# Spandan7724/Audio-Watermarking-Deep-Learning-Watermarks-for-Authenticating-Speech

Measured on AMD Instinct MI355X. Metric: 1-s@16kHz clips/sec (gen+det+loss fwd-bwd), higher is better.
Workload: dtype f32; 1 GPU; main16 train step: Generator+Detector+6 losses fwd-bwd + Adam, B=256 clips/GPU x 1 GPU, 1-s @ 16 kHz, message_bits=16 (BASELINE configs[2]); batch_per_gpu=256, global_batch=256, clip_len=16000, optimizer=fused flat Adam (wm_adam_step), parallelism=single

## Files before the change

### audio-watermarking-deep-learning-watermarks-for-authenticating-speech_amd/csrc/small_convs.hip

```cpp
#include "wm_common.hpp"
using namespace wm;

namespace {

__global__ __launch_bounds__(256) void stem_fwd_kernel(const float* __restrict__ s, const float* __restrict__ w,
                                                       const float* __restrict__ bias, float* __restrict__ y, int T) {
    __shared__ float ss[1024 + 8];
    __shared__ float ws[64 * 8];
    const int tilesPerClip = (T + 1023) / 1024;
    const int b = blockIdx.x / tilesPerClip, t0 = (blockIdx.x % tilesPerClip) * 1024;
    const float* sb = s + (size_t)b * T;
    for (int i = threadIdx.x; i < 1024 + 6; i += 256) {
        const int t = t0 - 3 + i;
        ss[i] = (t >= 0 && t < T) ? sb[t] : 0.f;
    }
    for (int i = threadIdx.x; i < 512; i += 256) {
        const int co = i >> 3, j = i & 7;
        ws[i] = (j < 7) ? w[co * 7 + j] : bias[co];
    }
    __syncthreads();
    const int t = t0 + 4 * threadIdx.x;
    if (t >= T) return;
    float v[10];
#pragma unroll
    for (int i = 0; i < 10; ++i) v[i] = ss[4 * threadIdx.x + i];
    float* yb = y + (size_t)b * 64 * T + t;
#pragma unroll 4
    for (int co = 0; co < 64; ++co) {
        const float* wc = ws + co * 8;
        float4 o = make_float4(wc[7], wc[7], wc[7], wc[7]);
#pragma unroll
        for (int j = 0; j < 7; ++j) {
            const float wj = wc[j];
            o.x = fmaf(wj, v[j], o.x);
            o.y = fmaf(wj, v[j + 1], o.y);
            o.z = fmaf(wj, v[j + 2], o.z);
            o.w = fmaf(wj, v[j + 3], o.w);
        }
        *reinterpret_cast<float4*>(yb + (size_t)co * T) = o;
    }
}

__global__ __launch_bounds__(256) void stem_bwd_kernel(const float* __restrict__ g, const float* __restrict__ s,
                                                       const float* __restrict__ w, float* __restrict__ ds,
                                                       float* __restrict__ partial, int B, int T, int nds) {
    constexpr int NT = 256, GS = NT + 8;
    extern __shared__ __align__(16) float smem[];
    float* gs = smem;
    float* ss = gs + 64 * GS;
    float* dsp = ss + NT + 40;
    const int tid = threadIdx.x, lane = tid & 63, wave = tid >> 6, half = lane >> 5, l31 = lane & 31;
    const int tilesPerClip = (T + NT - 1) / NT, ntiles = B * tilesPerClip;
    f32x16 acc[2];
#pragma unroll
    for (int r = 0; r < 16; ++r) { acc[0][r] = 0.f; acc[1][r] = 0.f; }
    float4 sg[16];
    float hg[2], sv[2];
    auto load_piece = [&](int tile, int p) {
        const int b = tile / tilesPerClip, t0 = (tile % tilesPerClip) * NT;
        const float* gb = g + (size_t)b * 64 * T;
        if (p < 16) {
            const int i = tid + p * 256, c = i >> 6, q = i & 63;
            sg[p] = *reinterpret_cast<const float4*>(gb + (size_t)c * T + min(t0 + 4 * q, T - 4));
            return;
        }
#pragma unroll
        for (int k = 0; k < 2; ++k) {
            const int i = min(tid + k * 256, 64 * 6 - 1), c = i / 6, h = i % 6;
            const int t = (h < 3) ? t0 - 3 + h : t0 + NT + (h - 3);
            hg[k] = gb[(size_t)c * T + min(max(t, 0), T - 1)];
            const int ts_ = t0 - 3 + tid + k * 256;
            sv[k] = s[(size_t)b * T + min(max(ts_, 0), T - 1)];
        }
    };
    auto load_tile = [&](int tile) {
#pragma unroll
        for (int p = 0; p <= 16; ++p) load_piece(tile, p);
    };
    auto write_tile = [&](int tile) {
        const int t0 = (tile % tilesPerClip) * NT;
#pragma unroll
        for (int k = 0; k < 16; ++k) {
            const int i = tid + k * 256, c = i >> 6, q = i & 63;
            float4 v = sg[k];
            if (t0 + 4 * q >= T) v = make_float4(0.f, 0.f, 0.f, 0.f);
            *reinterpret_cast<float4*>(gs + c * GS + 4 + 4 * q) = v;
        }
#pragma unroll
        for (int k = 0; k < 2; ++k) {
            const int i = tid + k * 256;
            if (i < 64 * 6) {
                const int c = i / 6, h = i % 6;
                const int t = (h < 3) ? t0 - 3 + h : t0 + NT + (h - 3);
                gs[c * GS + ((h < 3) ? 1 + h : 4 + NT + (h - 3))] = (t >= 0 && t < T) ? hg[k] : 0.f;
            }
            if (i < NT + 40) {
                const int ts_ = t0 - 3 + i;
                ss[i] = (i < NT + 6 && ts_ >= 0 && ts_ < T) ? sv[k] : 0.f;
            }
        }
    };
    int tile = blockIdx.x;
    if (tile < ntiles) load_tile(tile);
    __syncthreads();
    if (tile < ntiles) write_tile(tile);
    __syncthreads();
    while (tile < ntiles) {
        const int next = tile + gridDim.x, nextc = min(next, ntiles - 1);
        const int b = tile / tilesPerClip, t0 = (tile % tilesPerClip) * NT;
        {
            const float* ap = gs + l31 * GS + 4 + wave * 64 + half;
            const float* bp = ss + wave * 64 + half + l31;
            const bool tapcol = l31 < 7, onecol = l31 == 7;
#pragma unroll
            for (int k2 = 0; k2 < 32; ++k2) {
                if ((k2 & 1) == 0 || k2 == 31) load_piece(nextc, k2 == 31 ? 16 : k2 >> 1);
                const float sval = bp[2 * k2];
                const float bv = tapcol ? sval : (onecol ? 1.f : 0.f);
                acc[0] = mfma32(ap[2 * k2], bv, acc[0]);
                acc[1] = mfma32(ap[32 * GS + 2 * k2], bv, acc[1]);
            }
        }
        if (ds && b < nds) {
            const int cg = __builtin_amdgcn_readfirstlane(wave), tq = lane;
            float o0 = 0.f, o1 = 0.f, o2 = 0.f, o3 = 0.f;
#pragma unroll 4
            for (int cc = 0; cc < 16; ++cc) {
                const int co = cg * 16 + cc;
                const f32x4 ga = lds_read4(gs + co * GS + 4 * tq);
                const f32x4 gb4 = lds_read4(gs + co * GS + 4 * tq + 4);
                const f32x4 gc = lds_read4(gs + co * GS + 4 * tq + 8);
                const float* wc = w + co * 7;
                const float gv[10] = {ga.y, ga.z, ga.w, gb4.x, gb4.y, gb4.z, gb4.w, gc.x, gc.y, gc.z};
                const float wj[7] = {wc[0], wc[1], wc[2], wc[3], wc[4], wc[5], wc[6]};
#pragma unroll
                for (int j = 0; j < 7; ++j) {
                    o0 = fmaf(gv[6 - j], wj[j], o0); o1 = fmaf(gv[7 - j], wj[j], o1);
                    o2 = fmaf(gv[8 - j], wj[j], o2); o3 = fmaf(gv[9 - j], wj[j], o3);
                }
            }
            *reinterpret_cast<float4*>(dsp + cg * NT + 4 * tq) = make_float4(o0, o1, o2, o3);
        }
        __syncthreads();
        if (ds && b < nds) {
            const int t = t0 + tid;
            if (t < T) ds[(size_t)b * T + t] = (dsp[tid] + dsp[NT + tid]) + (dsp[2 * NT + tid] + dsp[3 * NT + tid]);
        }
        if (next < ntiles) write_tile(next);
        __syncthreads();
        tile = next;
    }
    float* red = gs;
    for (int wv = 0; wv < 4; ++wv) {
        if (wave == wv && l31 < 8) {
#pragma unroll
            for (int mt = 0; mt < 2; ++mt)
#pragma unroll
                for (int r = 0; r < 16; ++r) {
                    const int o = (mt * 32 + mfma_row(r, half)) * 8 + l31;
                    red[o] = (wv == 0) ? acc[mt][r] : red[o] + acc[mt][r];
                }
        }
        __syncthreads();
    }
    float* out = partial + (size_t)blockIdx.x * 512;
    for (int i = tid; i < 512; i += 256) out[i] = red[i];
}

__global__ __launch_bounds__(256) void reduce_partials_kernel(const float* __restrict__ partial, int nparts, int stride, int count,
                                                              float* __restrict__ out, int accumulate) {
    __shared__ double sq[4][64];
    const int i = blockIdx.x * 64 + (threadIdx.x & 63);
    const float s = (float)column_sum_d<4>(partial, nparts, (size_t)stride, i, i < count, sq);
    if (threadIdx.x < 64 && i < count) out[i] = accumulate ? out[i] + s : s;
}
__global__ __launch_bounds__(1024) void stem_reduce_kernel(const float* __restrict__ partial, int nparts, float* dw, float* db,
                                                           int accumulate) {
    __shared__ double sq[16][64];
    const int i = blockIdx.x * 64 + (threadIdx.x & 63);
    const float s = (float)column_sum_d<16>(partial, nparts, (size_t)512, i, true, sq);
    if (threadIdx.x >= 64) return;
    const int co = i >> 3, j = i & 7;
    float* dst = (j < 7) ? dw + co * 7 + j : db + co;
    *dst = accumulate ? *dst + s : s;
}

__global__ __launch_bounds__(256) void head1_fwd_kernel(const float* __restrict__ x, const float* __restrict__ w,
                                                        const float* __restrict__ bias, float* __restrict__ y, int T4,
                                                        int total4) {
    const int i = blockIdx.x * 256 + threadIdx.x;
    if (i >= total4) return;
    const int b = i / T4, q = i % T4;
    const float4* xb = reinterpret_cast<const float4*>(x) + (size_t)b * 64 * T4 + q;
    const float b0 = bias[0];
    float4 o = make_float4(b0, b0, b0, b0);
#pragma unroll 8
    for (int c = 0; c < 64; ++c) {
        const float4 v = xb[(size_t)c * T4];
        const float wc = w[c];
        o.x = fmaf(wc, v.x, o.x); o.y = fmaf(wc, v.y, o.y); o.z = fmaf(wc, v.z, o.z); o.w = fmaf(wc, v.w, o.w);
    }
    reinterpret_cast<float4*>(y)[i] = o;
}

template <bool MASK>
__global__ __launch_bounds__(256) void head1_tail_fwd_kernel(const float* __restrict__ x, const float* __restrict__ y2,
                                                             const float* __restrict__ scale, const float* __restrict__ shift,
                                                             float* __restrict__ out, unsigned* __restrict__ mask,
                                                             const float* __restrict__ w, const float* __restrict__ bias,
                                                             float* __restrict__ y, int T4) {
    const int tilesPerClip = (T4 + 255) / 256;
    const int b = blockIdx.x / tilesPerClip, q = (blockIdx.x % tilesPerClip) * 256 + (int)threadIdx.x;
    const bool ok = q < T4;
// ... 110 lines not shown
            unsigned* mrow = mask + ((size_t)b * 64 + lane) * nw;
            if (w0 < nw) mrow[w0] = mlo;
            if (w0 + 1 < nw) mrow[w0 + 1] = mhi;
        }
    } else {
#pragma unroll
        for (int c = 0; c < 64; ++c) v[c] = x[base + (size_t)c * T];
    }
    float sl = 0.f, sb = 0.f, yl = 0.f;
    long long msg = 0;
    if constexpr (LOSS) {
        if (b < BL) { msg = message[b]; yl = 1.f; }
    }
    auto one_output = [&](int o) {
        const float* wo = w + o * 64;
        float a0 = bias[o], a1 = 0.f, a2 = 0.f, a3 = 0.f;
#pragma unroll
        for (int c = 0; c < 64; c += 4) {
            a0 = fmaf(wo[c], v[c], a0); a1 = fmaf(wo[c + 1], v[c + 1], a1);
            a2 = fmaf(wo[c + 2], v[c + 2], a2); a3 = fmaf(wo[c + 3], v[c + 3], a3);
        }
        const float lg = (a0 + a1) + (a2 + a3);
        os[threadIdx.x * OS + o] = lg;
        if constexpr (LOSS) {
            const float term = valid ? bce_logits(lg, o == 0 ? yl : (float)((msg >> ((o - 1) & 63)) & 1)) : 0.f;
            if (o == 0) sl += term;
            else if (b < BL) sb += term;
        }
    };
    if constexpr (NOC > 0) {
#pragma unroll
        for (int o = 0; o < NOC; ++o) one_output(o);
    } else {
#pragma unroll 1
        for (int o = 0; o < no; ++o) {
            __builtin_amdgcn_sched_barrier(0);
            one_output(o);
        }
    }
    __syncthreads();
    const int nvalid = min(256, T - t0) * NO;
    float* yb = y + ((size_t)b * T + t0) * NO;
    for (int i = threadIdx.x; i < nvalid; i += 256) {
        if constexpr (NOC > 0) yb[i] = os[i];
        else { const int r = div_small(i, magic); yb[i] = os[r * OS + (i - r * NO)]; }
    }
    if constexpr (LOSS) {
        sl = block_sum<4>(sl, scratch);
        sb = block_sum<4>(sb, scratch + 4);
        if (threadIdx.x == 0) { partial[blockIdx.x] = sl; partial[gridDim.x + blockIdx.x] = sb; }
    }
}

template <int NOC, int NT, bool DL>
__global__ __launch_bounds__(256) void headN_bwd_kernel(const float* __restrict__ g, const float* __restrict__ x,
                                                        const float* __restrict__ w, float* __restrict__ dx,
                                                        float* __restrict__ partial, int B, int T, int no, unsigned magic,
                                                        const long long* __restrict__ message, const float* __restrict__ g_loc,
                                                        const float* __restrict__ g_bce, int BL) {
    constexpr int XS = 257, OB = 32 * NT, GS = OB + 1;
    constexpr int NOMAX = NOC > 0 ? NOC : OB;
    const int NO = NOC > 0 ? NOC : no;
    const int KS = (NO + 1) / 2;
    float kl = 0.f, kb = 0.f;
    if constexpr (DL) {
        kl = g_loc[0] / (float)((double)B * T);
        kb = (NO > 1) ? g_bce[0] / (float)((double)BL * T * (NO - 1)) : 0.f;
    }
    extern __shared__ __align__(16) float smem[];
    float* xs = smem;
    float* gsm = xs + 64 * XS;
    float* ws = gsm + 256 * GS;
    const int tid = threadIdx.x, lane = tid & 63, wave = tid >> 6, half = lane >> 5, l31 = lane & 31;
    for (int i = tid; i < OB * 64; i += 256) ws[i] = (i < NO * 64) ? w[i] : 0.f;
    for (int i = tid; i < 256 * GS; i += 256) gsm[i] = 0.f;
    const int tilesPerClip = (T + 255) / 256, ntiles = B * tilesPerClip;
    f32x16 accw[NT][2];
#pragma unroll
    for (int mt = 0; mt < NT; ++mt)
#pragma unroll
        for (int r = 0; r < 16; ++r) { accw[mt][0][r] = 0.f; accw[mt][1][r] = 0.f; }
    float accb = 0.f;
    constexpr int NG4 = (256 * NOMAX + 3) / 4, NGV = (NG4 + 255) / 256;
    float4 sx[16], sgv[NGV];
    auto load_piece = [&](int tile, int p) {
        const int b = tile / tilesPerClip, t0 = (tile % tilesPerClip) * 256;
        if (p < 16) {
            const int i = tid + p * 256, c = i >> 6, q = i & 63;
            sx[p] = *reinterpret_cast<const float4*>(x + ((size_t)b * 64 + c) * T + min(t0 + 4 * q, T - 4));
        } else {
            const float4* gb4 = reinterpret_cast<const float4*>(g + ((size_t)b * T + t0) * NO);
            const int lim4 = ((T - t0 < 256 ? T - t0 : 256) * NO) / 4;
            sgv[p - 16] = gb4[min(tid + (p - 16) * 256, lim4 - 1)];
        }
    };
    auto load_tile = [&](int tile) {
#pragma unroll
        for (int p = 0; p < 16 + NGV; ++p) load_piece(tile, p);
    };
    auto write_tile = [&](int tile) {
        const int t0 = (tile % tilesPerClip) * 256;
        const int nt = min(256, T - t0);
        const int row = tile / tilesPerClip;
        long long msg = 0;
        if constexpr (DL) msg = (row < BL) ? message[row] : 0;
        const float yl = row < BL ? 1.f : 0.f;
#pragma unroll
        for (int k = 0; k < 16; ++k) {
            const int i = tid + k * 256, c = i >> 6, q = i & 63;
            float4 v = sx[k];
            if (4 * q >= nt) v = make_float4(0.f, 0.f, 0.f, 0.f);
            float* d = xs + c * XS + 4 * q;
            d[0] = v.x; d[1] = v.y; d[2] = v.z; d[3] = v.w;
        }
#pragma unroll
        for (int k = 0; k < NGV; ++k) {
            const int f = tid + k * 256;
            if (f < NG4) {
                const float e[4] = {sgv[k].x, sgv[k].y, sgv[k].z, sgv[k].w};
#pragma unroll
                for (int j = 0; j < 4; ++j) {
                    const int i = 4 * f + j;
                    if (i < 256 * NO) {
                        const int r = NOC > 0 ? i / NO : div_small(i, magic), o = i - r * NO;
                        float val = e[j];
                        if constexpr (DL) {
                            if (o == 0) val = bce_logits_grad(val, yl, kl);
                            else val = (row < BL) ? bce_logits_grad(val, (float)((msg >> (o - 1)) & 1), kb) : 0.f;
                        }
                        gsm[r * GS + o] = (i < nt * NO) ? val : 0.f;
                    }
                }
            }
        }
    };
    int tile = blockIdx.x;
    if (tile < ntiles) load_tile(tile);
    __syncthreads();
    if (tile < ntiles) write_tile(tile);
    __syncthreads();
    while (tile < ntiles) {
        const int next = tile + gridDim.x, nextc = min(next, ntiles - 1);
        const int b = tile / tilesPerClip, t0 = (tile % tilesPerClip) * 256;
        const int nt = min(256, T - t0);
        {
            f32x16 acc[2][2];
#pragma unroll
            for (int mt = 0; mt < 2; ++mt)
#pragma unroll
                for (int n2 = 0; n2 < 2; ++n2)
#pragma unroll
                    for (int r = 0; r < 16; ++r) acc[mt][n2][r] = 0.f;
#pragma unroll
            for (int s = 0; s < (NOMAX + 1) / 2; ++s) {
                if (s < KS) {
                    const float a0 = ws[(2 * s + half) * 64 + l31], a1 = ws[(2 * s + half) * 64 + 32 + l31];
                    const float b0 = gsm[(wave * 64 + l31) * GS + 2 * s + half], b1 = gsm[(wave * 64 + 32 + l31) * GS + 2 * s + half];
                    acc[0][0] = mfma32(a0, b0, acc[0][0]); acc[0][1] = mfma32(a0, b1, acc[0][1]);
                    acc[1][0] = mfma32(a1, b0, acc[1][0]); acc[1][1] = mfma32(a1, b1, acc[1][1]);
                }
            }
            float* dxb = dx + (size_t)b * 64 * T + t0;
#pragma unroll
            for (int mt = 0; mt < 2; ++mt)
#pragma unroll
                for (int n2 = 0; n2 < 2; ++n2)
#pragma unroll
                    for (int r = 0; r < 16; ++r) {
                        const int c = mt * 32 + mfma_row(r, half), tt = wave * 64 + n2 * 32 + l31;
                        if (tt < nt) dxb[(size_t)c * T + tt] = acc[mt][n2][r];
                    }
        }
        {
            const float* ap = gsm + (wave * 64 + half) * GS + l31;
            const float* bp = xs + l31 * XS + wave * 64 + half;
#pragma unroll
            for (int s = 0; s < 32; ++s) {
                if (s < 16 + NGV) load_piece(nextc, s);
#pragma unroll
                for (int mt = 0; mt < NT; ++mt) {
                    const float a = ap[2 * s * GS + mt * 32];
                    accw[mt][0] = mfma32(a, bp[2 * s], accw[mt][0]);
                    accw[mt][1] = mfma32(a, bp[32 * XS + 2 * s], accw[mt][1]);
                }
            }
        }
        if ((tid & (OB - 1)) < NO) {
            const float* gp = gsm + (tid / OB) * OB * GS + (tid & (OB - 1));
#pragma unroll 8
            for (int tt = 0; tt < OB; ++tt) accb += gp[tt * GS];
        }
        __syncthreads();
        if (next < ntiles) write_tile(next);
        __syncthreads();
        tile = next;
    }
    __syncthreads();
    float* red = xs;
    for (int wv = 0; wv < 4; ++wv) {
        if (wave == wv) {
#pragma unroll
            for (int mt = 0; mt < NT; ++mt)
#pragma unroll
                for (int n2 = 0; n2 < 2; ++n2)
#pragma unroll
                    for (int r = 0; r < 16; ++r) {
                        const int o = mt * 32 + mfma_row(r, half), c = n2 * 32 + l31;
                        red[o * 64 + c] = (wv == 0) ? accw[mt][n2][r] : red[o * 64 + c] + accw[mt][n2][r];
                    }
        }
        __syncthreads();
    }
    float* out = partial + (size_t)blockIdx.x * (NO * 64 + NO);
    for (int i = tid; i < NO * 64; i += 256) out[i] = red[i];
    __syncthreads();
    red[tid] = ((tid & (OB - 1)) < NO) ? accb : 0.f;
    __syncthreads();
    if (tid < NO) {
        if constexpr (NT == 1)
            out[NO * 64 + tid] = ((red[tid] + red[32 + tid]) + (red[64 + tid] + red[96 + tid])) +
                                 ((red[128 + tid] + red[160 + tid]) + (red[192 + tid] + red[224 + tid]));
        else
            out[NO * 64 + tid] = (red[tid] + red[64 + tid]) + (red[128 + tid] + red[192 + tid]);
    }
}

}

extern "C" {

int wm_stem_fwd(const float* s, const float* w, const float* bias, float* y, int B, int T, hipStream_t stream) {
    if (T & 3) return (int)hipErrorInvalidValue;
    hipLaunchKernelGGL(stem_fwd_kernel, dim3(B * ((T + 1023) / 1024)), dim3(256), 0, stream, s, w, bias, y, T);
    WM_CHECK_LAUNCH();
    return 0;
}

#ifndef WM_STEM_WGS_PER_CU
#define WM_STEM_WGS_PER_CU 2
#endif
int wm_stem_bwd(const float* g, const float* s, const float* w, float* ds, float* partial, float* dw, float* db, int B,
                int T, int nds, int accumulate, hipStream_t stream) {
    if (T & 3) return (int)hipErrorInvalidValue;
    constexpr size_t lds = (size_t)(64 * 264 + 296 + 4 * 256) * sizeof(float);
    static wm::DevOnce attr_done;
    if (int rc = wm::lds_opt_in(reinterpret_cast<const void*>(stem_bwd_kernel), lds, attr_done)) return rc;
    const int ntiles = B * ((T + 255) / 256);
    const int grid = ntiles < WM_STEM_WGS_PER_CU * kNumCU ? ntiles : WM_STEM_WGS_PER_CU * kNumCU;
    hipLaunchKernelGGL(stem_bwd_kernel, dim3(grid), dim3(256), lds, stream, g, s, w, ds, partial, B, T, nds);
    WM_CHECK_LAUNCH();
    hipLaunchKernelGGL(stem_reduce_kernel, dim3(8), dim3(1024), 0, stream, (const float*)partial, grid, dw, db, accumulate);
    WM_CHECK_LAUNCH();
    return 0;
}

int wm_head1_fwd(const float* x, const float* w, const float* bias, float* y, int B, int T, hipStream_t stream) {
    if (T & 3) return (int)hipErrorInvalidValue;
    const int total4 = B * (T / 4);
    hipLaunchKernelGGL(head1_fwd_kernel, dim3((total4 + 255) / 256), dim3(256), 0, stream, x, w, bias, y, T / 4, total4);
    WM_CHECK_LAUNCH();
    return 0;
}

int wm_head1_tail_fwd(const float* x, const float* y2, const float* scale, const float* shift, const float* w, const float* bias,
                      float* out, void* mask, float* y, int B, int T, hipStream_t stream) {
    if ((T & 3) || B <= 0 || !y2 || !out) return (int)hipErrorInvalidValue;
    const int T4 = T / 4, grid = B * ((T4 + 255) / 256);
    if (mask) hipLaunchKernelGGL(head1_tail_fwd_kernel<true>, dim3(grid), dim3(256), 0, stream, x, y2, scale, shift, out, (unsigned*)mask, w, bias, y, T4);
    else hipLaunchKernelGGL(head1_tail_fwd_kernel<false>, dim3(grid), dim3(256), 0, stream, x, y2, scale, shift, out, (unsigned*)nullptr, w, bias, y, T4);
    WM_CHECK_LAUNCH();
    return 0;
}

int wm_head1_bwd(const float* g, const float* x, const float* w, float* dx, float* partial, float* dw, float* db, int B,
                 int T, int accumulate, hipStream_t stream) {
    if (T & 3) return (int)hipErrorInvalidValue;
    const int total4 = B * (T / 4);
    int grid = (total4 + 255) / 256;
    if (grid > 1024) grid = 1024;
    if (dx) hipLaunchKernelGGL(head1_bwd_kernel<true>, dim3(grid), dim3(256), 0, stream, g, x, w, dx, partial, T / 4, total4);
    else hipLaunchKernelGGL(head1_bwd_kernel<false>, dim3(grid), dim3(256), 0, stream, g, x, w, dx, partial, T / 4, total4);
    WM_CHECK_LAUNCH();
    hipLaunchKernelGGL(reduce_partials_kernel, dim3(1), dim3(256), 0, stream, (const float*)partial, grid, 65, 64, dw, accumulate);
    WM_CHECK_LAUNCH();
    hipLaunchKernelGGL(reduce_partials_kernel, dim3(1), dim3(256), 0, stream, (const float*)partial + 64, grid, 65, 1, db, accumulate);
    WM_CHECK_LAUNCH();
    return 0;
}

}

namespace {
struct HeadNFwd {
    const float *x, *y2, *scale, *shift, *w, *bias;
    float *out, *y, *partial;
    unsigned* mask;
    const long long* message;
    int BL, R, T, NO;
};
template <int NOC, bool TAIL, bool LOSS>
int launch_headN_fwd(const HeadNFwd& a, hipStream_t stream) {
    const size_t lds = (size_t)256 * (NOC > 0 ? NOC : (a.NO | 1)) * sizeof(float);
    if constexpr (NOC == 0) {
        static wm::DevOnce done;
        if (int rc = wm::lds_opt_in(reinterpret_cast<const void*>(headN_fwd_kernel<NOC, TAIL, LOSS>), 256 * 65 * sizeof(float), done)) return rc;
    }
    const unsigned magic = (unsigned)((0x100000000ull + a.NO - 1) / a.NO);
    hipLaunchKernelGGL((headN_fwd_kernel<NOC, TAIL, LOSS>), dim3(a.R * ((a.T + 255) / 256)), dim3(256), lds, stream, a.x, a.y2, a.scale,
                       a.shift, a.out, a.mask, a.w, a.bias, a.y, a.message, a.BL, a.partial, a.T, a.NO, magic);
    WM_CHECK_LAUNCH();
    return 0;
}
template <bool TAIL, bool LOSS>
int launch_headN_fwd_width(const HeadNFwd& a, hipStream_t stream) {
    if (a.NO == 17) return launch_headN_fwd<17, TAIL, LOSS>(a, stream);
    if (a.NO == 1) return launch_headN_fwd<1, TAIL, LOSS>(a, stream);
    return launch_headN_fwd<0, TAIL, LOSS>(a, stream);
}
}

extern "C" {

int wm_headN_fwd(const float* x, const float* w, const float* bias, float* y, int B, int T, int NO, hipStream_t stream) {
    if (NO < 1 || NO > 64 || B <= 0 || T <= 0) return (int)hipErrorInvalidValue;
    const HeadNFwd a{x, nullptr, nullptr, nullptr, w, bias, nullptr, y, nullptr, nullptr, nullptr, 0, B, T, NO};
    return launch_headN_fwd_width<false, false>(a, stream);
}

int wm_headN_tail_fwd(const float* x, const float* y2, const float* scale, const float* shift, const float* w, const float* bias,
                      const long long* message, int B, float* partial, float* loc_out, float* bce_out, float* out, void* mask,
                      float* logits, int R, int T, int NO, hipStream_t stream) {
    if (NO < 1 || NO > 64 || R <= 0 || T <= 0) return (int)hipErrorInvalidValue;
    if (y2 && (!scale || !shift || !out)) return (int)hipErrorInvalidValue;
    if (message && (B < 0 || B > R || !partial || !loc_out || (NO > 1 && !bce_out))) return (int)hipErrorInvalidValue;
    const HeadNFwd a{x, y2, scale, shift, w, bias, out, logits, partial, y2 ? (unsigned*)mask : nullptr, message, B, R, T, NO};
    const int rc = y2 ? (message ? launch_headN_fwd_width<true, true>(a, stream) : launch_headN_fwd_width<true, false>(a, stream))
                      : (message ? launch_headN_fwd_width<false, true>(a, stream) : launch_headN_fwd_width<false, false>(a, stream));
    if (rc || !message) return rc;
    const int grid = R * ((T + 255) / 256);
    WM_TRY((hipError_t)wm::launch_sum_scale2(partial, grid, 1.0 / ((double)R * T), loc_out, stream));
    if (NO > 1) WM_TRY((hipError_t)wm::launch_sum_scale2(partial + grid, grid, 1.0 / ((double)B * T * (NO - 1)), bce_out, stream));
    return 0;
}

}

namespace {
struct HeadNBwd {
    const float *g, *x, *w;
    float *dx, *partial;
    const long long* message;
    const float *g_loc, *g_bce;
    int BL, R, T, NO;
};
template <int NOC, int NT, bool DL>
int launch_headN_bwd(const HeadNBwd& a, int grid, hipStream_t stream) {
    constexpr size_t lds = (size_t)(64 * 257 + 256 * (32 * NT + 1) + 32 * NT * 64) * sizeof(float);
    static wm::DevOnce done;
    if (int rc = wm::lds_opt_in(reinterpret_cast<const void*>(headN_bwd_kernel<NOC, NT, DL>), lds, done)) return rc;
    const unsigned magic = a.NO > 1 ? (unsigned)((0x100000000ull + a.NO - 1) / a.NO) : 0u;
    hipLaunchKernelGGL((headN_bwd_kernel<NOC, NT, DL>), dim3(grid), dim3(256), lds, stream, a.g, a.x, a.w, a.dx, a.partial, a.R, a.T, a.NO,
                       magic, a.message, a.g_loc, a.g_bce, a.BL);
    WM_CHECK_LAUNCH();
    return 0;
}
template <bool DL>
int headN_bwd(const HeadNBwd& a, float* dw, float* db, int accumulate, hipStream_t stream) {
    const int NO = a.NO;
    if (NO < 1 || NO > 64) return (int)hipErrorInvalidValue;
    const int ntiles = a.R * ((a.T + 255) / 256);
    const int grid = ntiles < kNumCU ? ntiles : kNumCU;
    int rc;
    if (NO == 17) rc = launch_headN_bwd<17, 1, DL>(a, grid, stream);
    else if (NO == 1) rc = launch_headN_bwd<1, 1, DL>(a, grid, stream);
    else if (NO <= 32) rc = launch_headN_bwd<0, 1, DL>(a, grid, stream);
    else rc = launch_headN_bwd<0, 2, DL>(a, grid, stream);
    if (rc) return rc;
    const int n = NO * 64 + NO;
    hipLaunchKernelGGL(reduce_partials_kernel, dim3((NO * 64 + 63) / 64), dim3(256), 0, stream, (const float*)a.partial, grid, n, NO * 64, dw, accumulate);
    WM_CHECK_LAUNCH();
    hipLaunchKernelGGL(reduce_partials_kernel, dim3(1), dim3(256), 0, stream, (const float*)a.partial + NO * 64, grid, n, NO, db, accumulate);
    WM_CHECK_LAUNCH();
    return 0;
}
}

extern "C" {

int wm_headN_bwd(const float* g, const float* x, const float* w, float* dx, float* partial, float* dw, float* db, int B,
                 int T, int NO, int accumulate, hipStream_t stream) {
    const HeadNBwd a{g, x, w, dx, partial, nullptr, nullptr, nullptr, 0, B, T, NO};
    return headN_bwd<false>(a, dw, db, accumulate, stream);
}

int wm_headN_bwd_bce(const float* logits, const long long* message, const float* g_loc, const float* g_bce, const float* x,
                     const float* w, float* dx, float* partial, float* dw, float* db, int B, int R, int T, int NO, int accumulate,
                     hipStream_t stream) {
    if (!message || !g_loc || !g_bce || B < 0 || B > R) return (int)hipErrorInvalidValue;
    const HeadNBwd a{logits, x, w, dx, partial, message, g_loc, g_bce, B, R, T, NO};
    return headN_bwd<true>(a, dw, db, accumulate, stream);
}

}
```

### audio-watermarking-deep-learning-watermarks-for-authenticating-speech_amd/csrc/wm_common.hpp

```cpp
#pragma once
#include <hip/hip_runtime.h>
#include <stdint.h>
#include <atomic>

#define WM_CHECK_LAUNCH() do { hipError_t e_ = hipGetLastError(); if (e_ != hipSuccess) return (int)e_; } while (0)
#define WM_TRY(expr) do { hipError_t e_ = (expr); if (e_ != hipSuccess) return (int)e_; } while (0)

extern "C" int wm_gscale_absmax(const float* x, long long n, float* scratch, float log2_target, float* gscale, hipStream_t stream);

namespace wm {

struct DevOnce {
    std::atomic<unsigned long long> mask{0};
};
inline bool dev_done(const DevOnce& d) {
    int dev = 0;
    if (hipGetDevice(&dev) != hipSuccess) return false;
    return (d.mask.load(std::memory_order_acquire) >> (dev & 63)) & 1ull;
}
inline void dev_mark(DevOnce& d) {
    int dev = 0;
    if (hipGetDevice(&dev) != hipSuccess) return;
    d.mask.fetch_or(1ull << (dev & 63), std::memory_order_release);
}
inline int lds_opt_in(const void* kern, size_t lds, DevOnce& once) {
    if (dev_done(once)) return 0;
    WM_TRY(hipFuncSetAttribute(kern, hipFuncAttributeMaxDynamicSharedMemorySize, (int)lds));
    dev_mark(once);
    return 0;
}

inline bool overlap(const void* a, unsigned long long na, const void* b, unsigned long long nb) {
    const uintptr_t pa = (uintptr_t)a, pb = (uintptr_t)b;
    return pa < pb + nb && pb < pa + na;
}

typedef float f32x16 __attribute__((ext_vector_type(16)));
typedef float f32x4 __attribute__((ext_vector_type(4)));

typedef const volatile __attribute__((address_space(3))) f32x4 lds_f32x4_t;
__device__ __forceinline__ f32x4 lds_read4(const float* p) { return *(lds_f32x4_t*)p; }

constexpr int kWave = 64;
constexpr int kNumCU = 256;

__device__ __forceinline__ f32x16 mfma32(float a, float b, f32x16 c) {
    return __builtin_amdgcn_mfma_f32_32x32x2f32(a, b, c, 0, 0, 0);
}
__device__ __forceinline__ int mfma_row(int r, int half) { return (r & 3) + 8 * (r >> 2) + 4 * half; }

__device__ __forceinline__ float wave_sum(float v) {
#pragma unroll
    for (int o = 32; o > 0; o >>= 1) v += __shfl_xor(v, o);
    return v;
}
__device__ __forceinline__ float half_wave_sum(float v) {
#pragma unroll
    for (int o = 16; o > 0; o >>= 1) v += __shfl_xor(v, o);
    return v;
}
__device__ __forceinline__ float half_wave_transpose_sum32(float (&x)[32], int lane) {
#pragma unroll
    for (int s = 4; s >= 0; --s) {
        const int h = 1 << s;
        const bool up = (lane >> s) & 1;
#pragma unroll
        for (int i = 0; i < h; ++i) {
            const float keep = up ? x[i + h] : x[i];
            const float send = up ? x[i] : x[i + h];
            x[i] = keep + __shfl_xor(send, h);
        }
    }
    return x[0];
}
__device__ __forceinline__ float half_wave_transpose_sum16(float (&x)[16], int lane) {
#pragma unroll
    for (int s = 3; s >= 0; --s) {
        const int h = 1 << s;
        const bool up = (lane >> s) & 1;
#pragma unroll
        for (int i = 0; i < h; ++i) {
            const float keep = up ? x[i + h] : x[i];
            const float send = up ? x[i] : x[i + h];
            x[i] = keep + __shfl_xor(send, h);
        }
    }
    return x[0] + __shfl_xor(x[0], 16);
}
__device__ __forceinline__ double wave_sum_d(double v) {
#pragma unroll
    for (int o = 32; o > 0; o >>= 1) v += __shfl_xor(v, o);
    return v;
}

template <int NW>
__device__ __forceinline__ float block_sum(float v, float* scratch) {
    v = wave_sum(v);
    const int lane = threadIdx.x & 63, w = threadIdx.x >> 6;
    __syncthreads();
    if (lane == 0) scratch[w] = v;
// ... 165 lines not shown
```

### include/wm_hip.h

```cpp
#ifndef WM_HIP_H
#define WM_HIP_H

#ifdef __cplusplus
extern "C" {
#endif

typedef struct ihipStream_t* wm_stream_t;


int wm_pack_w64(const float* w, float* wp, int KW, int mode, wm_stream_t stream);

int wm_conv64(const float* x, const float* x2, const float* wp, const float* pa, const float* pb, const float* pc,
              const float* bias, const float* e1, const float* ea, const float* eb, float* y, float* stats,
              int B, int T, int KW, int pro, int epi, wm_stream_t stream);

int wm_pack_w64_bf(const float* w, void* wpb, int mode, wm_stream_t stream);
int wm_set_conv_bf_schedule(int schedule, wm_stream_t stream);
int wm_conv64_bf(const float* x, const float* x2, const void* wpb, const float* pa, const float* pb, const float* pc,
                 const float* bias, const float* e1, const float* ea, const float* eb, float* y, float* stats,
                 int B, int T, int pro, int epi, int arith, wm_stream_t stream);
int wm_conv64_bf_tail(const float* x, const float* y2, const void* wpb_h, const float* sc2, const float* sh2, const float* bias,
                      float* out, void* mask, float* y, float* stats, int B, int T, wm_stream_t stream);

int wm_conv64_bf_stem(const float* s, const float* stem_w, const float* stem_b, const void* wpb_h, const float* bias, float* y0,
// ... 24 lines not shown
                  int arith, const float* gscale, wm_stream_t stream);
int wm_pack_w64_h7(const float* w, void* wph, int mode, wm_stream_t stream);
int wm_gscale_absmax(const float* x, long long n, float* scratch, float log2_target, float* gscale, wm_stream_t stream);
int wm_gscale_from_max(const float* maxes, int n, float log2_target, float* gscale, wm_stream_t stream);
int wm_absmax_rows(const float* x, int rows, long long row_len, float* out, wm_stream_t stream);

int wm_wgrad64_bf7(const float* g, const float* x, const float* vec, float* partial, float* dw, float* dbias, int B, int T,
                   int xpro, int accumulate, int arith, const float* gscale, wm_stream_t stream);

int wm_wgrad64_bf(const float* g, const float* g2, const float* ga, const float* gb, const float* gc,
                  const float* x, const float* xa, const float* xb, float* partial, float* dw, float* dbias,
                  int B, int T, int gpro, int xpro, int accumulate, wm_stream_t stream);

int wm_wgrad64(const float* g, const float* g2, const float* ga, const float* gb, const float* gc,
               const float* x, const float* xa, const float* xb, float* partial, float* dw, float* dbias,
               int B, int T, int KW, int gpro, int xpro, int layout, int accumulate, wm_stream_t stream);

int wm_bn_finalize(const float* partials, int nparts, double count, const float* gamma, const float* beta,
                   float* running_mean, float* running_var, long long* num_batches_tracked, float momentum, float eps,
                   float* scale, float* shift, float* save_mean, float* save_invstd, wm_stream_t stream);
int wm_bn_eval_scale_shift(const float* gamma, const float* beta, const float* running_mean, const float* running_var,
                           float eps, float* scale, float* shift, wm_stream_t stream);
int wm_bn_add_relu(const float* x, const float* y2, const float* scale, const float* shift, float* out, int B, int T,
                   wm_stream_t stream);
int wm_relu_bwd_reduce(const float* g, const float* out, const float* y2, float* dz, float* partial, int B, int T,
                       wm_stream_t stream);
int wm_bn_add_relu_mask(const float* x, const float* y2, const float* scale, const float* shift, float* out, void* mask, int B, int T,
                        wm_stream_t stream);
int wm_relu_bwd_reduce_mask(const float* g, const void* mask, const float* y2, float* dz, float* partial, float* dzmax, int B, int T,
                            wm_stream_t stream);
int wm_relu_bwd_reduce_mask_r1(const float* g1, const float* w, const void* mask, const float* y2, float* partial, float* dzmax, int B,
                               int T, wm_stream_t stream);
int wm_bn_bwd_finalize(const float* partials, int nparts, double count, const float* gamma, const float* save_mean,
                       const float* save_invstd, float* A, float* Bc, float* Cc, float* dgamma, float* dbeta,
                       int accumulate, int eval_mode, const float* dzmax, int nmax, float* gscale, wm_stream_t stream);

int wm_stem_fwd(const float* s, const float* w, const float* bias, float* y, int B, int T, wm_stream_t stream);
int wm_stem_bwd(const float* g, const float* s, const float* w, float* ds, float* partial, float* dw, float* db, int B,
                int T, int nds, int accumulate, wm_stream_t stream);
int wm_head1_fwd(const float* x, const float* w, const float* bias, float* y, int B, int T, wm_stream_t stream);
int wm_head1_bwd(const float* g, const float* x, const float* w, float* dx, float* partial, float* dw, float* db, int B,
                 int T, int accumulate, wm_stream_t stream);
int wm_headN_fwd(const float* x, const float* w, const float* bias, float* y, int B, int T, int NO, wm_stream_t stream);
int wm_headN_bwd(const float* g, const float* x, const float* w, float* dx, float* partial, float* dw, float* db, int B,
                 int T, int NO, int accumulate, wm_stream_t stream);
int wm_head1_tail_fwd(const float* x, const float* y2, const float* scale, const float* shift, const float* w, const float* bias,
                      float* out, void* mask, float* y, int B, int T, wm_stream_t stream);
int wm_headN_tail_fwd(const float* x, const float* y2, const float* scale, const float* shift, const float* w, const float* bias,
                      const long long* message, int B, float* partial, float* loc_out, float* bce_out, float* out, void* mask,
                      float* logits, int R, int T, int NO, wm_stream_t stream);
int wm_headN_bwd_bce(const float* logits, const long long* message, const float* g_loc, const float* g_bce, const float* x,
                     const float* w, float* dx, float* partial, float* dw, float* db, int B, int R, int T, int NO, int accumulate,
                     wm_stream_t stream);

int wm_lstm_xproj(const float* x, const float* w_ih, const float* b_ih, const float* b_hh, float* xp, int B, int T,
                  wm_stream_t stream);
int wm_lstm_fwd(const float* xp, const float* w_hh, float* hout, float* gates, float* cst, int B, int T, wm_stream_t stream);
int wm_lstm_fwd_fused(const float* x, const float* w_ih, const float* b_ih, const float* b_hh, const float* w_hh,
                      float* hout, float* gates, float* cst, int B, int T, wm_stream_t stream);
int wm_set_lstm_fwd_wave_specialised(int on, wm_stream_t stream);
int wm_lstm_fwd_tail(const float* xres, const float* y2, const float* sc2, const float* sh2, float* out, void* mask, const float* w_ih,
                     const float* b_ih, const float* b_hh, const float* w_hh, float* hout, float* gates, float* cst, int B, int T,
                     wm_stream_t stream);
int wm_lstm_bwd(float* gates, const float* cst, const float* dh_out, const float* w_hh, int B, int T, wm_stream_t stream);
int wm_lstm_dx(const float* da, const float* w_ih, float* dx, int B, int T, wm_stream_t stream);
int wm_set_lstm_dx_bf16x6(int on, wm_stream_t stream);
int wm_lstm_bwd_fused(float* gates, const float* cst, const float* dh_out, const float* w_hh, const float* w_ih, float* dx,
                      int B, int T, wm_stream_t stream);
int wm_lstm_wgrad(const float* da, const float* x, const float* h, float* partial, float* dw_ih, float* dw_hh,
                  float* db_ih, float* db_hh, int B, int T, int accumulate, wm_stream_t stream);
int wm_lstm_bwd_wgrad(float* gates, const float* cst, const float* dh_out, const float* w_hh, const float* x, const float* h,
                      float* partial, float* dw_ih, float* dw_hh, float* db_ih, float* db_hh, int B, int T, int accumulate,
                      wm_stream_t stream);
int wm_lstm_bwd_wgrad_dx(const float* gates, const float* cst, const float* dh_out, const float* w_hh, const float* w_ih,
                         const float* x, const float* h, float* partial, float* dw_ih, float* dw_hh, float* db_ih, float* db_hh,
                         float* dx, int B, int T, int accumulate, wm_stream_t stream);

int wm_embed_gather(const float* table, const long long* message, float* vec, int B, int nrows, int* err, wm_stream_t stream);
int wm_embed_scatter_add(float* dtable, const long long* message, const float* dvec, int B, int nrows, wm_stream_t stream);
int wm_rowsum(const float* x, float* out, int rows, int T, wm_stream_t stream);

int wm_postproc_fwd(const float* d_in, const float* taps, int ntaps, float thr, float max_rms, float eps, int stages,
                    float* f_out, float* d_out, float* stats, int B, int T, wm_stream_t stream);
int wm_postproc_bwd(const float* g, const float* f_in, const float* stats, const float* taps, int ntaps, float thr,
                    float max_rms, int stages, float* d_raw, int B, int T, wm_stream_t stream);

int wm_mel_loss(const float* clean, const float* wm, const float* fb, const int* klo, const int* khi, const int* mlo,
                float* gframes, float* partial, float* loss_out, float* dsig, int B, int T, wm_stream_t stream);
int wm_loud_loss(const float* clean, const float* wm, float thresh, float* gframes, float* partial, float* loss_out,
                 float* dsig, int B, int T, wm_stream_t stream);
int wm_hf_penalty(const float* delta, int kcut, float* gframes, float* partial, float* loss_out, float* dsig, int B, int T,
                  wm_stream_t stream);

int wm_bce_fwd(const float* logits, const long long* message, float* partial, float* loc_out, float* bce_out, int B, int R,
               int T, int NO, wm_stream_t stream);
int wm_bce_bwd(const float* logits, const long long* message, const float* g_loc, const float* g_bce, float* dlogits, int B,
               int R, int T, int NO, wm_stream_t stream);
int wm_l1_fwd(const float* x, float* partial, float* out, long long n, wm_stream_t stream);
int wm_l1_bwd(const float* x, const float* g, float* dx, long long n, wm_stream_t stream);
int wm_adam_step(float* p, const float* g, float* m, float* v, long long n, double lr, double beta1, double beta2, double eps,
                 int step, wm_stream_t stream);

int wm_gconv(const float* x, const float* wp, const float* bias, const float* vec, const float* res, float* y, int NB,
             int Cin, int Lin, int K, int S, int P, int Mtot, int Nout, int st, int shp, int Cout, int Lout, int act,
             const float* x2, int Cin1, int nph, wm_stream_t stream);
int wm_gconv_h(const float* x, const void* wph, const float* bias, const float* vec, const float* res, float* y, int NB,
// ... 91 lines not shown
```

Measured before the change: 5777 clips/s.

## Rework stem and headN backward kernels with 16x16 MFMA and interleaved stores

```diff
diff --git a/audio-watermarking-deep-learning-watermarks-for-authenticating-speech_amd/csrc/small_convs.hip b/audio-watermarking-deep-learning-watermarks-for-authenticating-speech_amd/csrc/small_convs.hip
--- a/audio-watermarking-deep-learning-watermarks-for-authenticating-speech_amd/csrc/small_convs.hip
+++ b/audio-watermarking-deep-learning-watermarks-for-authenticating-speech_amd/csrc/small_convs.hip
@@ -41,6 +41,7 @@
     }
 }
 
+template <bool V1>
 __global__ __launch_bounds__(256) void stem_bwd_kernel(const float* __restrict__ g, const float* __restrict__ s,
                                                        const float* __restrict__ w, float* __restrict__ ds,
                                                        float* __restrict__ partial, int B, int T, int nds) {
@@ -50,10 +51,14 @@
     float* ss = gs + 64 * GS;
     float* dsp = ss + NT + 40;
     const int tid = threadIdx.x, lane = tid & 63, wave = tid >> 6, half = lane >> 5, l31 = lane & 31;
+    const int kq = lane >> 4, l15 = lane & 15;
     const int tilesPerClip = (T + NT - 1) / NT, ntiles = B * tilesPerClip;
     f32x16 acc[2];
+    f32x4 acc4[4];
 #pragma unroll
     for (int r = 0; r < 16; ++r) { acc[0][r] = 0.f; acc[1][r] = 0.f; }
+#pragma unroll
+    for (int mt = 0; mt < 4; ++mt) acc4[mt] = f32x4{0.f, 0.f, 0.f, 0.f};
     float4 sg[16];
     float hg[2], sv[2];
     auto load_piece = [&](int tile, int p) {
@@ -108,7 +113,7 @@
     while (tile < ntiles) {
         const int next = tile + gridDim.x, nextc = min(next, ntiles - 1);
         const int b = tile / tilesPerClip, t0 = (tile % tilesPerClip) * NT;
-        {
+        if constexpr (V1) {
             const float* ap = gs + l31 * GS + 4 + wave * 64 + half;
             const float* bp = ss + wave * 64 + half + l31;
             const bool tapcol = l31 < 7, onecol = l31 == 7;
@@ -119,6 +124,19 @@
                 const float bv = tapcol ? sval : (onecol ? 1.f : 0.f);
                 acc[0] = mfma32(ap[2 * k2], bv, acc[0]);
                 acc[1] = mfma32(ap[32 * GS + 2 * k2], bv, acc[1]);
+            }
+        } else {
+            const float* ap = gs + l15 * GS + 4 + wave * 64 + kq;
+            const float* bp = ss + wave * 64 + kq + l15;
+            const bool tapcol = l15 < 7, onecol = l15 == 7;
+#pragma unroll
+            for (int ks = 0; ks < 16; ++ks) {
+                load_piece(nextc, ks);
+                if (ks == 15) load_piece(nextc, 16);
+                const float sval = bp[4 * ks];
+                const float bv = tapcol ? sval : (onecol ? 1.f : 0.f);
+#pragma unroll
+                for (int mt = 0; mt < 4; ++mt) acc4[mt] = mfma16(ap[mt * 16 * GS + 4 * ks], bv, acc4[mt]);
             }
         }
         if (ds && b < nds) {
@@ -152,13 +170,22 @@
     }
     float* red = gs;
     for (int wv = 0; wv < 4; ++wv) {
-        if (wave == wv && l31 < 8) {
+        if (V1 && wave == wv && l31 < 8) {
 #pragma unroll
             for (int mt = 0; mt < 2; ++mt)
 #pragma unroll
                 for (int r = 0; r < 16; ++r) {
                     const int o = (mt * 32 + mfma_row(r, half)) * 8 + l31;
                     red[o] = (wv == 0) ? acc[mt][r] : red[o] + acc[mt][r];
+                }
+        }
+        if (!V1 && wave == wv && l15 < 8) {
+#pragma unroll
+            for (int mt = 0; mt < 4; ++mt)
+#pragma unroll
+                for (int r = 0; r < 4; ++r) {
+                    const int o = (mt * 16 + 4 * kq + r) * 8 + l15;
+                    red[o] = (wv == 0) ? acc4[mt][r] : red[o] + acc4[mt][r];
                 }
         }
         __syncthreads();
@@ -375,7 +402,7 @@
     }
 }
 
-template <int NOC, int NT, bool DL>
+template <int NOC, int NT, bool DL, bool V1>
 __global__ __launch_bounds__(256) void headN_bwd_kernel(const float* __restrict__ g, const float* __restrict__ x,
                                                         const float* __restrict__ w, float* __restrict__ dx,
                                                         float* __restrict__ partial, int B, int T, int no, unsigned magic,
@@ -406,6 +433,7 @@
     float accb = 0.f;
     constexpr int NG4 = (256 * NOMAX + 3) / 4, NGV = (NG4 + 255) / 256;
     float4 sx[16], sgv[NGV];
+    constexpr int NP = 16 + NGV, KSC = (NOMAX + 1) / 2, PD = V1 ? 0 : (KSC < NP ? KSC : NP);
     auto load_piece = [&](int tile, int p) {
         const int b = tile / tilesPerClip, t0 = (tile % tilesPerClip) * 256;
         if (p < 16) {
@@ -419,7 +447,7 @@
     };
     auto load_tile = [&](int tile) {
 #pragma unroll
-        for (int p = 0; p < 16 + NGV; ++p) load_piece(tile, p);
+        for (int p = 0; p < NP; ++p) load_piece(tile, p);
     };
     auto write_tile = [&](int tile) {
         const int t0 = (tile % tilesPerClip) * 256;
@@ -436,25 +464,55 @@
             float* d = xs + c * XS + 4 * q;
             d[0] = v.x; d[1] = v.y; d[2] = v.z; d[3] = v.w;
         }
-#pragma unroll
-        for (int k = 0; k < NGV; ++k) {
-            const int f = tid + k * 256;
-            if (f < NG4) {
-                const float e[4] = {sgv[k].x, sgv[k].y, sgv[k].z, sgv[k].w};
-#pragma unroll
-                for (int j = 0; j < 4; ++j) {
-                    const int i = 4 * f + j;
-                    if (i < 256 * NO) {
-                        const int r = NOC > 0 ? i / NO : div_small(i, magic), o = i - r * NO;
-                        float val = e[j];
-                        if constexpr (DL) {
-                            if (o == 0) val = bce_logits_grad(val, yl, kl);
-                            else val = (row < BL) ? bce_logits_grad(val, (float)((msg >> (o - 1)) & 1), kb) : 0.f;
+        if constexpr (V1) {
+#pragma unroll
+            for (int k = 0; k < NGV; ++k) {
+                const int f = tid + k * 256;
+                if (f < NG4) {
+                    const float e[4] = {sgv[k].x, sgv[k].y, sgv[k].z, sgv[k].w};
+#pragma unroll
+                    for (int j = 0; j < 4; ++j) {
+                        const int i = 4 * f + j;
+                        if (i < 256 * NO) {
+                            const int r = NOC > 0 ? i / NO : div_small(i, magic), o = i - r * NO;
+                            float val = e[j];
+                            if constexpr (DL) {
+                                if (o == 0) val = bce_logits_grad(val, yl, kl);
+                                else val = (row < BL) ? bce_logits_grad(val, (float)((msg >> (o - 1)) & 1), kb) : 0.f;
+                            }
+                            gsm[r * GS + o] = (i < nt * NO) ? val : 0.f;
                         }
-                        gsm[r * GS + o] = (i < nt * NO) ? val : 0.f;
                     }
                 }
             }
+        } else {
+            float val[NGV][4];
+            int adr[NGV][4];
+#pragma unroll
+            for (int k = 0; k < NGV; ++k) {
+                const int f = tid + k * 256;
+                const float e[4] = {sgv[k].x, sgv[k].y, sgv[k].z, sgv[k].w};
+#pragma unroll
+                for (int j = 0; j < 4; ++j) {
+                    const int i = 4 * f + j, ic = min(i, 256 * NO - 1);
+                    const int r = NOC > 0 ? ic / NO : div_small(ic, magic), o = ic - r * NO;
+                    float v = e[j];
+                    if constexpr (DL) {
+                        const bool loc = o == 0;
+                        const float y = loc ? yl : (float)((msg >> ((o - 1) & 63)) & 1);
+                        v = bce_logits_grad(v, y, loc ? kl : kb);
+                        v = (loc || row < BL) ? v : 0.f;
+                    }
+                    val[k][j] = (i < nt * NO) ? v : 0.f;
+                    asm volatile("" : "+v"(val[k][j]));
+                    adr[k][j] = (f < NG4 && i < 256 * NO) ? r * GS + o : -1;
+                }
+            }
+#pragma unroll
+            for (int k = 0; k < NGV; ++k)
+#pragma unroll
+                for (int j = 0; j < 4; ++j)
+                    if (adr[k][j] >= 0) gsm[adr[k][j]] = val[k][j];
         }
     };
     int tile = blockIdx.x;
@@ -466,8 +524,24 @@
         const int next = tile + gridDim.x, nextc = min(next, ntiles - 1);
         const int b = tile / tilesPerClip, t0 = (tile % tilesPerClip) * 256;
         const int nt = min(256, T - t0);
+        f32x16 acc[2][2];
+        float* dxb = dx + (size_t)b * 64 * T + t0;
+        const wm_srd_t sdx = make_srd(dx + (size_t)b * 64 * T, (size_t)64 * T * sizeof(float));
+        unsigned vdx[2];
+#pragma unroll
+        for (int n2 = 0; n2 < 2; ++n2) {
+            const int tt = wave * 64 + n2 * 32 + l31;
+            vdx[n2] = tt < nt ? (unsigned)(4 * half * T + t0 + tt) * 4u : 0xffffffffu;
+        }
+        auto store_dx = [&](int mt, int n2, int r) {
+            if constexpr (V1) {
+                const int c = mt * 32 + mfma_row(r, half), tt = wave * 64 + n2 * 32 + l31;
+                if (tt < nt) dxb[(size_t)c * T + tt] = acc[mt][n2][r];
+            } else {
+                buf_store(sdx, acc[mt][n2][r], vdx[n2], (unsigned)((mt * 32 + mfma_row(r, 0)) * T) * 4u);
+            }
+        };
         {
-            f32x16 acc[2][2];
 #pragma unroll
             for (int mt = 0; mt < 2; ++mt)
 #pragma unroll
@@ -475,46 +549,55 @@
 #pragma unroll
                     for (int r = 0; r < 16; ++r) acc[mt][n2][r] = 0.f;
 #pragma unroll
-            for (int s = 0; s < (NOMAX + 1) / 2; ++s) {
+            for (int s = 0; s < KSC; ++s) {
+                if (s < PD) load_piece(nextc, s);
                 if (s < KS) {
                     const float a0 = ws[(2 * s + half) * 64 + l31], a1 = ws[(2 * s + half) * 64 + 32 + l31];
                     const float b0 = gsm[(wave * 64 + l31) * GS + 2 * s + half], b1 = gsm[(wave * 64 + 32 + l31) * GS + 2 * s + half];
                     acc[0][0] = mfma32(a0, b0, acc[0][0]); acc[0][1] = mfma32(a0, b1, acc[0][1]);
                     acc[1][0] = mfma32(a1, b0, acc[1][0]); acc[1][1] = mfma32(a1, b1, acc[1][1]);
                 }
-            }
-            float* dxb = dx + (size_t)b * 64 * T + t0;
-#pragma unroll
-            for (int mt = 0; mt < 2; ++mt)
-#pragma unroll
-                for (int n2 = 0; n2 < 2; ++n2)
-#pragma unroll
-                    for (int r = 0; r < 16; ++r) {
-                        const int c = mt * 32 + mfma_row(r, half), tt = wave * 64 + n2 * 32 + l31;
-                        if (tt < nt) dxb[(size_t)c * T + tt] = acc[mt][n2][r];
-                    }
+                if constexpr (!V1) __builtin_amdgcn_sched_barrier(0);
+            }
+            if constexpr (V1) {
+#pragma unroll
+                for (int mt = 0; mt < 2; ++mt)
+#pragma unroll
+                    for (int n2 = 0; n2 < 2; ++n2)
+#pragma unroll
+                        for (int r = 0; r < 16; ++r) store_dx(mt, n2, r);
+            }
         }
         {
             const float* ap = gsm + (wave * 64 + half) * GS + l31;
             const float* bp = xs + l31 * XS + wave * 64 + half;
+            const float* gp = gsm + (tid / OB) * OB * GS + (tid & (OB - 1));
+            static_assert(V1 || OB == 32, "one step of the bias sums per k-step of the dw product");
 #pragma unroll
             for (int s = 0; s < 32; ++s) {
-                if (s < 16 + NGV) load_piece(nextc, s);
+                if (PD + s < NP) load_piece(nextc, PD + s);
+                if constexpr (!V1) {
+                    store_dx(s >> 4, (s >> 3) & 1, (2 * s) & 15);
+                    store_dx(s >> 4, (s >> 3) & 1, (2 * s + 1) & 15);
+                    accb += gp[s * GS];
+                }
 #pragma unroll
                 for (int mt = 0; mt < NT; ++mt) {
                     const float a = ap[2 * s * GS + mt * 32];
                     accw[mt][0] = mfma32(a, bp[2 * s], accw[mt][0]);
                     accw[mt][1] = mfma32(a, bp[32 * XS + 2 * s], accw[mt][1]);
                 }
-            }
-        }
-        if ((tid & (OB - 1)) < NO) {
+                if constexpr (!V1) __builtin_amdgcn_sched_barrier(0);
+            }
+        }
+        if (V1 && (tid & (OB - 1)) < NO) {
             const float* gp = gsm + (tid / OB) * OB * GS + (tid & (OB - 1));
 #pragma unroll 8
             for (int tt = 0; tt < OB; ++tt) accb += gp[tt * GS];
         }
         __syncthreads();
-        if (next < ntiles) write_tile(next);
+        if constexpr (!V1) write_tile(nextc);
+        else if (next < ntiles) write_tile(next);
         __syncthreads();
         tile = next;
     }
@@ -562,15 +645,21 @@
 #ifndef WM_STEM_WGS_PER_CU
 #define WM_STEM_WGS_PER_CU 2
 #endif
+static int g_small_bwd_v1 = 0;
+int wm_set_small_bwd_v1(int on, hipStream_t) { g_small_bwd_v1 = on ? 1 : 0; return 0; }
+
 int wm_stem_bwd(const float* g, const float* s, const float* w, float* ds, float* partial, float* dw, float* db, int B,
                 int T, int nds, int accumulate, hipStream_t stream) {
     if (T & 3) return (int)hipErrorInvalidValue;
     constexpr size_t lds = (size_t)(64 * 264 + 296 + 4 * 256) * sizeof(float);
-    static wm::DevOnce attr_done;
-    if (int rc = wm::lds_opt_in(reinterpret_cast<const void*>(stem_bwd_kernel), lds, attr_done)) return rc;
+    static wm::DevOnce attr_done[2];
+    const int v1 = g_small_bwd_v1;
+    const void* kernel = v1 ? reinterpret_cast<const void*>(stem_bwd_kernel<true>) : reinterpret_cast<const void*>(stem_bwd_kernel<false>);
+    if (int rc = wm::lds_opt_in(kernel, lds, attr_done[v1])) return rc;
     const int ntiles = B * ((T + 255) / 256);
     const int grid = ntiles < WM_STEM_WGS_PER_CU * kNumCU ? ntiles : WM_STEM_WGS_PER_CU * kNumCU;
-    hipLaunchKernelGGL(stem_bwd_kernel, dim3(grid), dim3(256), lds, stream, g, s, w, ds, partial, B, T, nds);
+    if (v1) hipLaunchKernelGGL(stem_bwd_kernel<true>, dim3(grid), dim3(256), lds, stream, g, s, w, ds, partial, B, T, nds);
+    else hipLaunchKernelGGL(stem_bwd_kernel<false>, dim3(grid), dim3(256), lds, stream, g, s, w, ds, partial, B, T, nds);
     WM_CHECK_LAUNCH();
     hipLaunchKernelGGL(stem_reduce_kernel, dim3(8), dim3(1024), 0, stream, (const float*)partial, grid, dw, db, accumulate);
     WM_CHECK_LAUNCH();
@@ -676,16 +765,22 @@
     const float *g_loc, *g_bce;
     int BL, R, T, NO;
 };
+template <int NOC, int NT, bool DL, bool V1>
+int launch_headN_bwd_build(const HeadNBwd& a, int grid, hipStream_t stream) {
+    constexpr size_t lds = (size_t)(64 * 257 + 256 * (32 * NT + 1) + 32 * NT * 64) * sizeof(float);
+    static wm::DevOnce done;
+    if (int rc = wm::lds_opt_in(reinterpret_cast<const void*>(headN_bwd_kernel<NOC, NT, DL, V1>), lds, done)) return rc;
+    const unsigned magic = a.NO > 1 ? (unsigned)((0x100000000ull + a.NO - 1) / a.NO) : 0u;
+    hipLaunchKernelGGL((headN_bwd_kernel<NOC, NT, DL, V1>), dim3(grid), dim3(256), lds, stream, a.g, a.x, a.w, a.dx, a.partial, a.R, a.T,
+                       a.NO, magic, a.message, a.g_loc, a.g_bce, a.BL);
+    WM_CHECK_LAUNCH();
+    return 0;
+}
 template <int NOC, int NT, bool DL>
 int launch_headN_bwd(const HeadNBwd& a, int grid, hipStream_t stream) {
-    constexpr size_t lds = (size_t)(64 * 257 + 256 * (32 * NT + 1) + 32 * NT * 64) * sizeof(float);
-    static wm::DevOnce done;
-    if (int rc = wm::lds_opt_in(reinterpret_cast<const void*>(headN_bwd_kernel<NOC, NT, DL>), lds, done)) return rc;
-    const unsigned magic = a.NO > 1 ? (unsigned)((0x100000000ull + a.NO - 1) / a.NO) : 0u;
-    hipLaunchKernelGGL((headN_bwd_kernel<NOC, NT, DL>), dim3(grid), dim3(256), lds, stream, a.g, a.x, a.w, a.dx, a.partial, a.R, a.T, a.NO,
-                       magic, a.message, a.g_loc, a.g_bce, a.BL);
-    WM_CHECK_LAUNCH();
-    return 0;
+    if constexpr (NT == 2) return launch_headN_bwd_build<NOC, NT, DL, true>(a, grid, stream);
+    else return (g_small_bwd_v1 || (size_t)a.T * 256 >= 0xfffff000ull) ? launch_headN_bwd_build<NOC, NT, DL, true>(a, grid, stream)
+                                                                      : launch_headN_bwd_build<NOC, NT, DL, false>(a, grid, stream);
 }
 template <bool DL>
 int headN_bwd(const HeadNBwd& a, float* dw, float* db, int accumulate, hipStream_t stream) {
diff --git a/audio-watermarking-deep-learning-watermarks-for-authenticating-speech_amd/csrc/wm_common.hpp b/audio-watermarking-deep-learning-watermarks-for-authenticating-speech_amd/csrc/wm_common.hpp
--- a/audio-watermarking-deep-learning-watermarks-for-authenticating-speech_amd/csrc/wm_common.hpp
+++ b/audio-watermarking-deep-learning-watermarks-for-authenticating-speech_amd/csrc/wm_common.hpp
@@ -46,6 +46,9 @@
 
 __device__ __forceinline__ f32x16 mfma32(float a, float b, f32x16 c) {
     return __builtin_amdgcn_mfma_f32_32x32x2f32(a, b, c, 0, 0, 0);
+}
+__device__ __forceinline__ f32x4 mfma16(float a, float b, f32x4 c) {
+    return __builtin_amdgcn_mfma_f32_16x16x4f32(a, b, c, 0, 0, 0);
 }
 __device__ __forceinline__ int mfma_row(int r, int half) { return (r & 3) + 8 * (r >> 2) + 4 * half; }
 
diff --git a/include/wm_hip.h b/include/wm_hip.h
--- a/include/wm_hip.h
+++ b/include/wm_hip.h
@@ -100,6 +100,7 @@
 int wm_headN_bwd_bce(const float* logits, const long long* message, const float* g_loc, const float* g_bce, const float* x,
                      const float* w, float* dx, float* partial, float* dw, float* db, int B, int R, int T, int NO, int accumulate,
                      wm_stream_t stream);
+int wm_set_small_bwd_v1(int on, wm_stream_t stream);
 
 int wm_lstm_xproj(const float* x, const float* w_ih, const float* b_ih, const float* b_hh, float* xp, int B, int T,
                   wm_stream_t stream);
```

Result: no change. 5814 clips/s (median of 6 runs) (+0.6%).
